# wasiahmad/context_attentive_ir

Measured on AMD Instinct MI355X. Metric: ranked (query,doc) pairs/sec, higher is better.
Workload: dtype f32; 1 GPU; cars, batch=16 sessions x session_len 7 x 10 candidates, q_len=4, doc_len=64, emb_dim=300, vocab=100000, f32, full-length Zipf ids; macro_batch=8, lanes=4, batches_in_flight=32, hipgraph=True, parallelism=single GPU, world_size=1

## Files before the change

### context_attentive_ir_amd/csrc/cars_attn.hip

```cpp
#include <algorithm>
#include <mutex>
#include <type_traits>
#include "common.hpp"

namespace nir {

typedef _Float16 f16x8 __attribute__((ext_vector_type(8)));
typedef __fp16 fp16x2_t __attribute__((ext_vector_type(2)));
typedef float f32x4 __attribute__((ext_vector_type(4)));

constexpr int AP_D = 256;
constexpr int AP_ROWS = 64, AP_RT = 4, AP_CT = 4, AP_S = AP_D / 32;
constexpr int AP_KG = AP_ROWS * 8 + 32;
constexpr int AP_PLANE_HALVES = 2 * AP_S * 4 * AP_KG;
constexpr int AP_RED_FLOATS = 4 * 16 * AP_D;
constexpr size_t AP_LDS = (size_t)(AP_PLANE_HALVES * 2 > AP_RED_FLOATS * 4 ? AP_PLANE_HALVES * 2 : AP_RED_FLOATS * 4) + (4 * 64 + 64) * 4;

#define AP_MMA(ACC, A, W) asm volatile("v_mfma_f32_16x16x32_f16 %0, %1, %2, %0" : "+a"(ACC) : "v"(A), "v"(W))
#define AP_MMA_DRAIN() asm volatile("s_nop 15\n\ts_nop 15" ::: "memory")

__device__ __forceinline__ void ap_mma_n(int n, f32x4 (&acc)[AP_CT][AP_RT], f32x4 (&acx)[AP_CT][AP_RT], const f16x8 (&af)[AP_RT][2],
                                         const f16x8 (&w)[AP_CT][2]) {
    const int j = n / (3 * AP_RT), ph = (n / AP_RT) % 3, i = n % AP_RT;
    if (ph == 0) AP_MMA(acx[j][i], af[i][1], w[j][0]);
// ... 8 lines not shown
    if (T >= 16) v = fmaxf(v, dpp_mov<0x140>(v));
    if (T >= 32) v = fmaxf(v, __shfl_xor(v, 16));
    if (T >= 64) v = fmaxf(v, __shfl_xor(v, 32));
    return v;
}
__device__ __forceinline__ float ap_group_sum(float v, int T) {
    v += dpp_mov<0xB1>(v);
    v += dpp_mov<0x4E>(v);
    if (T >= 8) v += dpp_mov<0x141>(v);
    if (T >= 16) v += dpp_mov<0x140>(v);
    if (T >= 32) v += __shfl_xor(v, 16);
    if (T >= 64) v += __shfl_xor(v, 32);
    return v;
}

struct AttnPoolArgs {
    const float* h;
    const _Float16* wf;
    const float *b0, *w3, *b3;
    const int64_t* lens;
    float* pooled;
    int64_t M;
    int T, logT;
    int io_prio;
};

__global__ __launch_bounds__(256, 1) void attn_pool_fused_kernel(AttnPoolArgs p) {
    extern __shared__ __attribute__((aligned(16))) unsigned short asm_[];
    unsigned short* Pp = asm_;
    float* rowpart = reinterpret_cast<float*>(asm_ + (AP_LDS - (4 * 64 + 64) * 4) / 2);
    float* prob = rowpart + 4 * 64;
    constexpr int KG = AP_KG;
    const int tid = threadIdx.x, lane = tid & 63, wave = tid >> 6;
    const int g = lane >> 4, c16 = lane & 15;
    const int T = p.T;
    const int64_t row0 = (int64_t)blockIdx.x * AP_ROWS, nrows = p.M * T;

    const _Float16* wp = p.wf + ((int64_t)(AP_CT * wave) * 2 * 64 + lane) * 8;
    constexpr int WSTEP = 16 * 2 * 64 * 8;
    f16x8 w[AP_CT][2], wb[AP_CT][2], afa[AP_RT][2], afb[AP_RT][2];
    {
        float4 hv[16];
#pragma unroll
        for (int j = 0; j < 16; ++j) {
            int64_t r = row0 + wave + 4 * j;
            r = r < nrows ? r : nrows - 1;
            hv[j] = *reinterpret_cast<const float4*>(p.h + r * AP_D + 4 * lane);
// ... 125 lines not shown
            a.x = fmaf(pr, hv[j].x, a.x); a.y = fmaf(pr, hv[j].y, a.y); a.z = fmaf(pr, hv[j].z, a.z); a.w = fmaf(pr, hv[j].w, a.w);
            if (((j + 1) & (per - 1)) == 0) {
                red[(wave * RS + (j >> (p.logT - 2))) * 64 + lane] = a;
                a = make_float4(0.f, 0.f, 0.f, 0.f);
            }
        }
        __syncthreads();
        for (int idx = tid; idx < RS * 64; idx += 256) {
            const int q = idx >> 6, c = idx & 63;
            const int64_t seq = (row0 >> p.logT) + q;
            if (seq < p.M) {
                const float4 a0 = red[(0 * RS + q) * 64 + c], a1 = red[(1 * RS + q) * 64 + c], a2 = red[(2 * RS + q) * 64 + c],
                             a3 = red[(3 * RS + q) * 64 + c];
                float4 o;
                o.x = (a0.x + a1.x) + (a2.x + a3.x); o.y = (a0.y + a1.y) + (a2.y + a3.y);
                o.z = (a0.z + a1.z) + (a2.z + a3.z); o.w = (a0.w + a1.w) + (a2.w + a3.w);
                *reinterpret_cast<float4*>(p.pooled + seq * AP_D + 4 * c) = o;
            }
        }
    }
}

#ifdef AP_TIMING
__device__ long long ap_dbg[16];
#define AP_T(I) if (blockIdx.x == 7 && lane == 0 && it == 5) ap_dbg[I] = __builtin_readcyclecounter();
#else
#define AP_T(I)
#endif
constexpr int AP2_KG = AP_ROWS * 8;
constexpr int AP2_PLANE_HALVES = 2 * AP_S * 4 * AP2_KG;
constexpr size_t AP2_LDS = (size_t)2 * AP2_PLANE_HALVES * 2 + (2 * 4 * 64 + 4 * 64 + 2 * AP_D) * 4;

template <bool ONE, bool ROW1>
__device__ __forceinline__ void ap2_mma_n(int n, f32x4 (&acc)[AP_CT][AP_RT], f32x4 (&acx)[AP_CT][AP_RT], const f16x8 (&af)[AP_RT][2],
                                          const f16x8 (&w)[AP_CT][2]) {
    const int i = n / (3 * AP_CT), ph = (n / AP_CT) % 3, j = n % AP_CT;
    if (ph == 2) AP_MMA(acc[j][i], af[i][0], w[j][0]);
    else if (ONE) return;
    else if (ph == 0) { if (!ROW1) AP_MMA(acx[j][i], af[i][1], w[j][0]); }
    else AP_MMA(acx[j][i], af[i][0], w[j][1]);
}

#ifndef AP_FMAMIX
#define AP_FMAMIX 1
#endif
__device__ __forceinline__ void ap_fma_mix(float4& a, const uint2 u, const float s) {
    asm volatile("v_fma_mix_f32 %0, %1, %2, %0 op_sel:[0,0,0] op_sel_hi:[1,0,0]" : "+v"(a.x) : "v"(u.x), "v"(s));
    asm volatile("v_fma_mix_f32 %0, %1, %2, %0 op_sel:[1,0,0] op_sel_hi:[1,0,0]" : "+v"(a.y) : "v"(u.x), "v"(s));
    asm volatile("v_fma_mix_f32 %0, %1, %2, %0 op_sel:[0,0,0] op_sel_hi:[1,0,0]" : "+v"(a.z) : "v"(u.y), "v"(s));
    asm volatile("v_fma_mix_f32 %0, %1, %2, %0 op_sel:[1,0,0] op_sel_hi:[1,0,0]" : "+v"(a.w) : "v"(u.y), "v"(s));
}

template <bool ONE, int IN>
__global__ __launch_bounds__(512, 1) void attn_pool_pipe_kernel(AttnPoolArgs p, int64_t ntiles) {
    constexpr bool IN16 = IN == 1;
    constexpr bool ROW1 = ONE || IN16;
    extern __shared__ __attribute__((aligned(16))) unsigned short asm2_[];
    constexpr int KG = AP2_KG, PH = AP2_PLANE_HALVES;
    float* rowpart = reinterpret_cast<float*>(asm2_ + 2 * PH);
    float* probw = rowpart + 2 * 4 * 64;
    float* bw = probw + 4 * 64;
    const int tid = threadIdx.x, lane = tid & 63, wave = tid >> 6, w4 = wave & 3;
    if (tid < AP_D) bw[tid] = p.b0[tid] * 2.8853900817779268f;
    else bw[tid] = p.w3[tid - AP_D];
    __syncthreads();
    const bool mma_role = wave < 4;
    const int g = lane >> 4, c16 = lane & 15;
    const int T = p.T;
    const int64_t nrows = p.M * T;
    const int64_t G = gridDim.x;
    const int64_t nk = (ntiles - blockIdx.x + G - 1) / G;

    if (mma_role) {
        __builtin_amdgcn_s_setprio(3);
        const _Float16* wbase = p.wf + (int64_t)(AP_CT * __builtin_amdgcn_readfirstlane(w4)) * 2 * 64 * 8;
        uint32_t wlane = (uint32_t)lane * 16u;
        auto ldw = [&](int off_halves) {
            return *reinterpret_cast<const f16x8*>(reinterpret_cast<const char*>(wbase + off_halves) + (uint64_t)wlane);
        };
        constexpr int WSTEP = 16 * 2 * 64 * 8;
        const int foff_e = g * KG + (c16 ^ (2 * (g >> 1))) * 8, foff_o = g * KG + (c16 ^ (4 + 2 * (g >> 1))) * 8;
        f16x8 wa[AP_CT][2], wb[AP_CT][2], af[AP_RT][2];
        f32x4 acc[AP_CT][AP_RT], acx[AP_CT][AP_RT];
#pragma unroll
        for (int j = 0; j < AP_CT; ++j) {
            wa[j][0] = ldw((j * 2) * 512);
            wa[j][1] = ONE ? wa[j][0] : ldw((j * 2 + 1) * 512);
        }
        for (int64_t it = 0; it < nk + 2; ++it) {
            if (w4 == 0) { AP_T(0) }
            if (it >= 1 && it <= nk) {
                const unsigned short* Pp = asm2_ + ((it - 1) & 1) * PH;
                float* rp = rowpart + ((it - 1) & 1) * 4 * 64;
#pragma unroll
                for (int j = 0; j < AP_CT; ++j)
#pragma unroll
                    for (int i = 0; i < AP_RT; ++i) {
                        acc[j][i] = f32x4{0.f, 0.f, 0.f, 0.f};
                        acx[j][i] = f32x4{0.f, 0.f, 0.f, 0.f};
                    }
#pragma unroll
                for (int i = 0; i < AP_RT - 1; ++i) {
                    af[i][0] = *reinterpret_cast<const f16x8*>(Pp + foff_e + i * 128);
                    af[i][1] = *reinterpret_cast<const f16x8*>(Pp + AP_S * 4 * KG + foff_e + i * 128);
                }
#define AP2_STEP(S, WC, WN, LAST, ODD)                                                    \
                {                                                                         \
                    const int sn_ = ((S) + 1) & (AP_S - 1);                               \
                    asm volatile("" : "+v"(wlane));                                       \
                    const unsigned short* pc_ = Pp + (S) * 4 * KG + ((ODD) ? foff_o : foff_e);  \
                    const unsigned short* pn_ = Pp + sn_ * 4 * KG + ((ODD) ? foff_e : foff_o);  \
                    _Pragma("clang loop unroll(full)") for (int n_ = 0; n_ < 3 * AP_RT * AP_CT; ++n_) { \
                        ap2_mma_n<ONE, ROW1>(n_, acc, acx, af, WC);                             \
                        if (n_ % 6 == 2 && n_ / 6 < 2 * AP_CT && !(ONE && ((n_ / 6) & 1))) {  \
                            asm volatile("" ::"v"(WN[(n_ / 6) >> 1][(n_ / 6) & 1]));      \
                            WN[(n_ / 6) >> 1][(n_ / 6) & 1] = ldw(sn_ * WSTEP + (n_ / 6) * 512);  \
                        }                                                                 \
                        if (n_ == 7 || n_ == 8) {                                         \
                            asm volatile("" ::"v"(af[3][n_ - 7]));                        \
                            af[3][n_ - 7] = *reinterpret_cast<const f16x8*>(pc_ + (n_ - 7) * AP_S * 4 * KG + 3 * 128); \
                        }                                                                 \
                        if (!(LAST) && n_ >= 19 && (n_ - 19) % 12 < 2 && (n_ - 19) / 12 < AP_RT - 1) { \
                            asm volatile("" ::"v"(af[(n_ - 19) / 12][(n_ - 19) % 12]));   \
                            af[(n_ - 19) / 12][(n_ - 19) % 12] =                          \
                                *reinterpret_cast<const f16x8*>(pn_ + ((n_ - 19) % 12) * AP_S * 4 * KG + ((n_ - 19) / 12) * 128); \
                        }                                                                 \
                        __builtin_amdgcn_sched_barrier(0);                                \
                    }                                                                     \
                    _Pragma("unroll") for (int j_ = 0; j_ < AP_CT; ++j_) asm volatile("" ::"v"(WC[j_][0]), "v"(WC[j_][1])); \
                    _Pragma("unroll") for (int i_ = 0; i_ < AP_RT; ++i_) asm volatile("" ::"v"(af[i_][0]), "v"(af[i_][1])); \
                }
#pragma unroll 1
                for (int s = 0; s < AP_S - 2; s += 2) {
                    AP2_STEP(s, wa, wb, 0, 0)
                    AP2_STEP(s + 1, wb, wa, 0, 1)
                }
                AP2_STEP(AP_S - 2, wa, wb, 0, 0)
                AP2_STEP(AP_S - 1, wb, wa, 1, 1)
                if (w4 == 0) { AP_T(1) }
                AP_MMA_DRAIN();
                {
                    constexpr float C2 = 2.8853900817779268f;
                    float rs[AP_RT][4], bzv[AP_CT], w3v[AP_CT];
#pragma unroll
                    for (int j = 0; j < AP_CT; ++j) {
                        const int col = 64 * w4 + 16 * j + c16;
                        bzv[j] = bw[col];
                        w3v[j] = bw[AP_D + col];
                    }
                    const float r0 = -0.5f * ((w3v[0] + w3v[1]) + (w3v[2] + w3v[3]));
#pragma unroll
                    for (int i = 0; i < AP_RT; ++i)
#pragma unroll
                        for (int r = 0; r < 4; ++r) rs[i][r] = r0;
#pragma unroll
                    for (int j = 0; j < AP_CT; ++j) {
#pragma unroll
                        for (int i = 0; i < AP_RT; ++i)
#pragma unroll
                            for (int r = 0; r < 4; ++r) {
                                const float z = fmaf(fmaf(acx[j][i][r], 1.0f / 2048.0f, acc[j][i][r]), C2, bzv[j]);
                                rs[i][r] = fmaf(w3v[j], __builtin_amdgcn_rcpf(1.0f + __builtin_amdgcn_exp2f(z)), rs[i][r]);
                            }
                    }
#pragma unroll
                    for (int i = 0; i < AP_RT; ++i)
#pragma unroll
                        for (int r = 0; r < 4; ++r) {
                            float v = rs[i][r];
                            v += dpp_mov<0xB1>(v);
                            v += dpp_mov<0x4E>(v);
                            v += dpp_mov<0x141>(v);
                            v += dpp_mov<0x140>(v);
                            if (c16 == 0) rp[w4 * 64 + 16 * i + 4 * g + r] = -2.0f * v;
                        }
                }
            }
            if (w4 == 0) { AP_T(2) }
            __syncthreads();
            if (w4 == 0) { AP_T(3) }
        }
    } else {
        if (p.io_prio) __builtin_amdgcn_s_setprio(2);
        float* pw = probw + w4 * 64;
        const int sub = lane >> 4, per = T / 4;
        const int col = 64 * w4 + 4 * c16;
        const int poff = ((col >> 5) * 4 + ((col >> 3) & 3)) * KG + (col & 7);
        const int xq = c16 >> 3, sx = sub ^ (2 * ((c16 >> 2) & 1));
        const int roff_e = (4 * xq + sx) * 8, roff_o = (4 * (1 ^ xq) + sx) * 8;
        float4 ld[IN16 ? 1 : 16];
        uint2 ld16[IN16 ? 16 : 1];
        const float b3v = p.b3[0];
        int len_ld = T, len_1 = T, len_2 = T;
        auto load_rows = [&](int64_t k) {
            const int64_t row0 = (blockIdx.x + k * G) * AP_ROWS;
            {
                const int64_t seq = (row0 + lane) >> p.logT;
                len_ld = T;
                if (p.lens) len_ld = (int)p.lens[seq < p.M ? seq : p.M - 1];
            }
#pragma unroll
            for (int q = 0; q < 16; ++q) {
                int64_t r = row0 + 4 * q + sub;
                r = r < nrows ? r : nrows - 1;
                if (IN16) ld16[q] = *reinterpret_cast<const uint2*>(reinterpret_cast<const _Float16*>(p.h) + r * AP_D + col);
                else ld[q] = *reinterpret_cast<const float4*>(p.h + r * AP_D + col);
            }
        };
        if (nk > 0) load_rows(0);
        for (int64_t it = 0; it < nk + 2; ++it) {
            unsigned short* Pb = asm2_ + (it & 1) * PH + poff;
            unsigned short* Pbe = Pb + roff_e;
            unsigned short* Pbo = Pb + roff_o;
            if (w4 == 0) { AP_T(4) }
            if (it >= 2) {
                const int64_t rowS = (blockIdx.x + (it - 2) * G) * AP_ROWS;
                const float* rp = rowpart + (it & 1) * 4 * 64;
                {
                    const int64_t r = rowS + lane;
                    const int64_t seq = r >> p.logT;
                    const int t = (int)(r - seq * T);
                    int len = len_2;
                    len = len < 0 ? 0 : (len > T ? T : len);
                    const bool ok = seq < p.M && t < len;
                    const float lg = (rp[lane] + rp[64 + lane]) + (rp[128 + lane] + rp[192 + lane]) + b3v;
                    const float mx = ap_group_max(ok ? lg : -INFINITY, T);
                    const float e = ok ? __expf(lg - mx) : 0.f;
                    const float den = ap_group_sum(e, T);
                    pw[lane] = e / den;
                    asm volatile("s_waitcnt lgkmcnt(0)" ::: "memory");
                }
                if (w4 == 0) { AP_T(8) }
                float4 a = make_float4(0.f, 0.f, 0.f, 0.f);
#pragma unroll
                for (int hb = 0; hb < 2; ++hb) {
                    uint2 u1[8], u2[ROW1 ? 1 : 8];
                    float prr[8];
#pragma unroll
                    for (int q8 = 0; q8 < 8; ++q8) {
                        const int row = 4 * (8 * hb + q8) + sub;
                        const unsigned short* src = ((q8 & 1) ? Pbo : Pbe) + ((8 * hb + q8) >> 1) * 64;
                        u1[q8] = *reinterpret_cast<const uint2*>(src);
                        if (!ROW1) u2[q8] = *reinterpret_cast<const uint2*>(src + AP_S * 4 * KG);
                        prr[q8] = pw[row];
                    }
#pragma unroll
                    for (int q8 = 0; q8 < 8; ++q8) {
                        const int q = 8 * hb + q8;
                        const fp16x2_t a01 = __builtin_bit_cast(fp16x2_t, u1[q8].x), a23 = __builtin_bit_cast(fp16x2_t, u1[q8].y);
                        const float pr = prr[q8];
#if AP_FMAMIX
                        (void)a01; (void)a23;
                        ap_fma_mix(a, u1[q8], pr);
                        if (!ROW1) ap_fma_mix(a, u2[q8], pr * (1.0f / 2048.0f));
#else
                        if (ROW1) {
                            a.x = fmaf(pr, (float)a01[0], a.x);
                            a.y = fmaf(pr, (float)a01[1], a.y);
                            a.z = fmaf(pr, (float)a23[0], a.z);
                            a.w = fmaf(pr, (float)a23[1], a.w);
                        } else {
                            const fp16x2_t b01 = __builtin_bit_cast(fp16x2_t, u2[q8].x), b23 = __builtin_bit_cast(fp16x2_t, u2[q8].y);
                            a.x = fmaf(pr, fmaf((float)b01[0], 1.0f / 2048.0f, (float)a01[0]), a.x);
                            a.y = fmaf(pr, fmaf((float)b01[1], 1.0f / 2048.0f, (float)a01[1]), a.y);
                            a.z = fmaf(pr, fmaf((float)b23[0], 1.0f / 2048.0f, (float)a23[0]), a.z);
                            a.w = fmaf(pr, fmaf((float)b23[1], 1.0f / 2048.0f, (float)a23[1]), a.w);
                        }
#endif
                        if (((q + 1) & (per - 1)) == 0) {
                            a.x += __shfl_xor(a.x, 16); a.y += __shfl_xor(a.y, 16); a.z += __shfl_xor(a.z, 16); a.w += __shfl_xor(a.w, 16);
                            a.x += __shfl_xor(a.x, 32); a.y += __shfl_xor(a.y, 32); a.z += __shfl_xor(a.z, 32); a.w += __shfl_xor(a.w, 32);
                            const int64_t seq = (rowS >> p.logT) + (q >> (p.logT - 2));
                            if (sub == 0 && seq < p.M) *reinterpret_cast<float4*>(p.pooled + seq * AP_D + col) = a;
                            a = make_float4(0.f, 0.f, 0.f, 0.f);
                        }
                    }
                }
            }
            if (w4 == 0) { AP_T(5) }
            if (it < nk) {
#pragma unroll
                for (int q = 0; q < 16; ++q) {
                    unsigned short* d = ((q & 1) ? Pbo : Pbe) + (q >> 1) * 64;
                    if (IN16) {
                        *reinterpret_cast<uint2*>(d) = ld16[q];
                        continue;
                    }
                    const float4 v = ld[q];
                    if (IN == 2) {
                        *reinterpret_cast<uint2*>(d) = make_uint2(__float_as_uint(v.x), __float_as_uint(v.y));
                        *reinterpret_cast<uint2*>(d + AP_S * 4 * KG) = make_uint2(__float_as_uint(v.z), __float_as_uint(v.w));
                        continue;
                    }
                    const fp16x2_t a01 = __builtin_amdgcn_cvt_pkrtz(v.x, v.y), a23 = __builtin_amdgcn_cvt_pkrtz(v.z, v.w);
                    *reinterpret_cast<uint2*>(d) = make_uint2(__builtin_bit_cast(unsigned, a01), __builtin_bit_cast(unsigned, a23));
                    if (!ONE) {
                        const fp16x2_t b01 = __builtin_amdgcn_cvt_pkrtz((v.x - (float)a01[0]) * 2048.0f, (v.y - (float)a01[1]) * 2048.0f);
                        const fp16x2_t b23 = __builtin_amdgcn_cvt_pkrtz((v.z - (float)a23[0]) * 2048.0f, (v.w - (float)a23[1]) * 2048.0f);
                        *reinterpret_cast<uint2*>(d + AP_S * 4 * KG) = make_uint2(__builtin_bit_cast(unsigned, b01), __builtin_bit_cast(unsigned, b23));
                    }
                }
                if (w4 == 0) { AP_T(6) }
                len_2 = len_1;
                len_1 = len_ld;
                if (it + 1 < nk) load_rows(it + 1);
            } else {
                len_2 = len_1;
            }
            if (w4 == 0) { AP_T(7) }
            __syncthreads();
        }
    }
}

#ifdef AP_TIMING
}
extern "C" int nir_debug_attn_timing(long long* out16) { return (int)hipMemcpyFromSymbol(out16, HIP_SYMBOL(nir::ap_dbg), sizeof(long long) * 16); }
namespace nir {
#endif

bool attn_pool_fused_usable(int D, int T) { return D == AP_D && (T == 4 || T == 8 || T == 16 || T == 32 || T == 64); }

static int ap_cu_count() {
    static const int ncu = [] {
        int dev = 0;
        hipDeviceProp_t prop;
        return (hipGetDevice(&dev) == hipSuccess && hipGetDeviceProperties(&prop, dev) == hipSuccess && prop.multiProcessorCount > 0)
                   ? prop.multiProcessorCount : 256;
    }();
    return ncu;
}
bool attn_pool_pipe_selected(int64_t M, int T) {
    const int64_t tiles = (M * T + AP_ROWS - 1) / AP_ROWS;
    const int pipe = tun(g_tun.attn_unfused_pipe);
    return (tiles >= 2 * (int64_t)ap_cu_count() && pipe == 0) || pipe == 2;
}

int launch_attn_pool_fused(const float* h, const void* wfrag, const float* b0, const float* w3, const float* b3, const int64_t* lens, int64_t M,
                           int T, float* pooled, int one_term, hipStream_t st, int in_f16) {
    NIR_REQUIRE(h && wfrag && b0 && w3 && b3 && pooled && attn_pool_fused_usable(AP_D, T), "attn_pool_fused: bad args (T=%d)", T);
    if (M == 0) return 0;
    AttnPoolArgs a;
    a.h = h; a.wf = (const _Float16*)wfrag; a.b0 = b0; a.w3 = w3; a.b3 = b3; a.lens = lens; a.pooled = pooled; a.M = M; a.T = T; a.logT = __builtin_ctz((unsigned)T);
    a.io_prio = tun(g_tun.attn_io_prio);
    static std::once_flag once;
    std::call_once(once, [] { (void)hipFuncSetAttribute((const void*)attn_pool_fused_kernel, hipFuncAttributeMaxDynamicSharedMemorySize, (int)AP_LDS); });
    const int64_t tiles = (M * T + AP_ROWS - 1) / AP_ROWS;
    const bool pipe_sel = attn_pool_pipe_selected(M, T);
    const char* pname = !pipe_sel ? "attn_pool_fused_kernel" : in_f16 == 1 ? "attn_pool_pipe_kernel<true,1>" : in_f16 == 3 ? "attn_pool_pipe_kernel<false,1>" :
                        in_f16 == 2 ? "attn_pool_pipe_kernel<false,2>" :
                        one_term ? "attn_pool_pipe_kernel<true,0>" : "attn_pool_pipe_kernel<false,0>";
    ProfScope ps(prof_shape_name(pname, M * T, AP_D, AP_D), st);
    static std::once_flag once2;
    std::call_once(once2, [] {
        (void)hipFuncSetAttribute((const void*)attn_pool_pipe_kernel<false, 0>, hipFuncAttributeMaxDynamicSharedMemorySize, (int)AP2_LDS);
        (void)hipFuncSetAttribute((const void*)attn_pool_pipe_kernel<false, 2>, hipFuncAttributeMaxDynamicSharedMemorySize, (int)AP2_LDS);
        (void)hipFuncSetAttribute((const void*)attn_pool_pipe_kernel<true, 0>, hipFuncAttributeMaxDynamicSharedMemorySize, (int)AP2_LDS);
        (void)hipFuncSetAttribute((const void*)attn_pool_pipe_kernel<true, 1>, hipFuncAttributeMaxDynamicSharedMemorySize, (int)AP2_LDS);
        (void)hipFuncSetAttribute((const void*)attn_pool_pipe_kernel<false, 1>, hipFuncAttributeMaxDynamicSharedMemorySize, (int)AP2_LDS);
    });
    const int ncu = ap_cu_count();
    if (pipe_sel) {
        const dim3 grid((unsigned)std::min<int64_t>(tiles, ncu));
        NIR_REQUIRE(in_f16 != 2 || !one_term, "attn_pool_fused: term-pair rows come from the fp32-accurate encoder (two terms)");
        if (in_f16 == 1) hipLaunchKernelGGL((attn_pool_pipe_kernel<true, 1>), grid, dim3(512), AP2_LDS, st, a, tiles);
        else if (in_f16 == 3) hipLaunchKernelGGL((attn_pool_pipe_kernel<false, 1>), grid, dim3(512), AP2_LDS, st, a, tiles);
        else if (in_f16 == 2) hipLaunchKernelGGL((attn_pool_pipe_kernel<false, 2>), grid, dim3(512), AP2_LDS, st, a, tiles);
// ... 12 lines not shown
```

### context_attentive_ir_amd/csrc/common.hpp

```cpp
#pragma once
#include <hip/hip_runtime.h>
#include <stdint.h>
#include <stdio.h>
#include <stdarg.h>
#include <atomic>
#include "../../include/neuroir_hip.h"

namespace nir {

void set_error(const char* fmt, ...);

#define NIR_REQUIRE(cond, ...)                 \
    do {                                       \
        if (!(cond)) {                         \
            nir::set_error(__VA_ARGS__);       \
            return NIR_ERR_BAD_ARG;            \
        }                                      \
    } while (0)

#define NIR_CHECK_LAUNCH(name)                                                      \
    do {                                                                            \
        hipError_t e__ = hipGetLastError();                                         \
        if (e__ != hipSuccess) {                                                    \
            nir::set_error("%s: launch failed: %s", name, hipGetErrorString(e__)); \
// ... 10 lines not shown
struct ProfScope {
    void* rec;
    hipStream_t st;
    ProfScope(const char* name, hipStream_t stream);
    ~ProfScope();
};

const char* prof_shape_name(const char* base, long long M, long long N, long long K);

struct ForkJoin {
    hipStream_t main, side;
    hipEvent_t ev_fork, ev_join;
    bool ok, open;
    explicit ForkJoin(hipStream_t main_stream);
    ~ForkJoin() { if (open) join(); }
    void fork();
    void join();
};

extern unsigned long long* g_debug_buf;
int batches_in_flight(hipStream_t st);

struct Tunables {
    std::atomic<int> no_fork, lstm_mfma16, lstm_s, debug, exact_f32, duet_unfused, attn_unfused, attn_unfused_pipe, duet_rows64, attn_fp32_rows, attn_io_prio, cl_poll_limit;
};
extern Tunables g_tun;
inline int tun(const std::atomic<int>& a) { return a.load(std::memory_order_relaxed); }

constexpr int WAVE = 64;

template <int CTRL>
__device__ __forceinline__ float dpp_mov(float v) {
    return __builtin_bit_cast(float, __builtin_amdgcn_update_dpp(0, __builtin_bit_cast(int, v), CTRL, 0xF, 0xF, true));
}
__device__ __forceinline__ float readlane_f(float v, int lane) {
    return __builtin_bit_cast(float, __builtin_amdgcn_readlane(__builtin_bit_cast(int, v), lane));
}
__device__ __forceinline__ float wave_sum(float v) {
    v += dpp_mov<0xB1>(v);
    v += dpp_mov<0x4E>(v);
    v += dpp_mov<0x141>(v);
    v += dpp_mov<0x140>(v);
    return (readlane_f(v, 0) + readlane_f(v, 16)) + (readlane_f(v, 32) + readlane_f(v, 48));
}
__device__ __forceinline__ float wave_max(float v) {
    v = fmaxf(v, dpp_mov<0xB1>(v));
    v = fmaxf(v, dpp_mov<0x4E>(v));
// ... 94 lines not shown
```

### context_attentive_ir_amd/csrc/core.hip

```cpp
#include "common.hpp"
#include <string.h>
#include <stdlib.h>
#include <atomic>
#include <map>
#include <mutex>
#include <string>
#include <vector>

namespace nir {
static thread_local char g_err[512] = "";
void set_error(const char* fmt, ...) {
    va_list ap;
    va_start(ap, fmt);
    vsnprintf(g_err, sizeof(g_err), fmt, ap);
    va_end(ap);
}
}

namespace nir {
struct ProfRec { const char* name; hipEvent_t a, b; };
static std::mutex g_prof_mu;
static std::vector<ProfRec*> g_prof;
static std::atomic<int> g_prof_on{0};

// ... 113 lines not shown
static int env_flag(const char* name) { return getenv(name) ? 1 : 0; }
Tunables g_tun{{env_flag("NIR_NO_FORK")}, {env_int("NIR_LSTM_MFMA16", -1)}, {env_int("NIR_LSTM_S", 0)}, {env_flag("NIR_DEBUG")},
               {env_flag("NIR_EXACT_F32")}};
}
extern "C" int nir_set_stream_batches_in_flight(nir_stream_t stream, int n) {
    std::lock_guard<std::mutex> lk(nir::g_bif_mu);
    if (n < 1) nir::g_bif_map.erase((hipStream_t)stream);
    else nir::g_bif_map[(hipStream_t)stream] = n;
    nir::g_bif_streams.store((int)nir::g_bif_map.size());
    return 0;
}
static const bool g_tunables_mutable = getenv("NIR_DEBUG_TUNABLES") != nullptr;
extern "C" int nir_debug_set_tunable(const char* name, int value) {
    using namespace nir;
    if (!name) return NIR_ERR_BAD_ARG;
    if (!g_tunables_mutable) {
        set_error("nir_debug_set_tunable('%s'): the switches are frozen at load time; set NIR_DEBUG_TUNABLES=1 before loading the library (debug / test processes only)", name);
        return NIR_ERR_BAD_ARG;
    }
    struct { const char* n; std::atomic<int>* a; } tab[] = {
        {"no_fork", &g_tun.no_fork}, {"lstm_mfma16", &g_tun.lstm_mfma16}, {"lstm_s", &g_tun.lstm_s}, {"debug", &g_tun.debug},
        {"exact_f32", &g_tun.exact_f32}, {"duet_unfused", &g_tun.duet_unfused}, {"attn_unfused", &g_tun.attn_unfused},
        {"attn_unfused_pipe", &g_tun.attn_unfused_pipe}, {"duet_rows64", &g_tun.duet_rows64}, {"attn_fp32_rows", &g_tun.attn_fp32_rows},
        {"attn_io_prio", &g_tun.attn_io_prio}, {"cl_poll_limit", &g_tun.cl_poll_limit}};
    for (auto& t : tab)
        if (!strcmp(t.n, name)) { t.a->store(value); return 0; }
    set_error("nir_debug_set_tunable: unknown tunable '%s'", name);
    return NIR_ERR_BAD_ARG;
}
extern "C" int nir_debug_set_buffer(void* dev_u64) { nir::g_debug_buf = (unsigned long long*)dev_u64; return 0; }

__global__ void clock_probe_kernel(unsigned long long* out, int iters, float* sink) {
    extern __shared__ float probe_lds[];
    unsigned long long c0 = clock64(), w0 = wall_clock64();
    if (iters < 0) probe_lds[threadIdx.x] = 1.f;
    float a = threadIdx.x * 1e-9f, b = 1.000001f;
    for (int i = 0; i < iters; ++i) a = fmaf(a, b, 1e-7f);
    unsigned long long c1 = clock64(), w1 = wall_clock64();
    if (a == 123.456f) sink[0] = a;
    if (blockIdx.x == 0 && threadIdx.x == 0) { out[0] = c1 - c0; out[1] = w1 - w0; }
    if (threadIdx.x == 0 && blockIdx.x < 2048) {
        out[2 + 3 * blockIdx.x] = w0;
        out[3 + 3 * blockIdx.x] = w1;
        out[4 + 3 * blockIdx.x] = __builtin_amdgcn_s_getreg(63492);
    }
}
extern "C" int nir_debug_clock_probe(void* out, int iters, int blocks, void* sink, nir_stream_t stream) {
// ... 198 lines not shown
```

Before: 8.325 million pairs/s.

## Restructure attention-pool pipe kernel into two symmetric ping-pong wave groups

The pipelined attention-pool kernel previously split waves into dedicated MFMA waves and I/O/softmax waves. Now two groups of four waves each own one LDS plane and alternate tiles. Each group runs MFMA, scoring, softmax, pooling and staging of its next tile, with an LDS atomic counter for intra-group sync and shared barriers between groups. The goal is to overlap one group's MFMA phase with the other's memory and epilogue work without a fixed role imbalance. The cost is more complex synchronisation and a higher register load per wave. The unused io_prio tunable is also removed.

```diff
diff --git a/context_attentive_ir_amd/csrc/cars_attn.hip b/context_attentive_ir_amd/csrc/cars_attn.hip
--- a/context_attentive_ir_amd/csrc/cars_attn.hip
+++ b/context_attentive_ir_amd/csrc/cars_attn.hip
@@ -54,7 +54,6 @@
     float* pooled;
     int64_t M;
     int T, logT;
-    int io_prio;
 };
 
 __global__ __launch_bounds__(256, 1) void attn_pool_fused_kernel(AttnPoolArgs p) {
@@ -226,14 +225,16 @@
 }
 
 #ifdef AP_TIMING
-__device__ long long ap_dbg[16];
-#define AP_T(I) if (blockIdx.x == 7 && lane == 0 && it == 5) ap_dbg[I] = __builtin_readcyclecounter();
+__device__ long long ap_dbg[32];
+#define AP_T(I) if (blockIdx.x == 7 && lane == 0 && w4 == 0 && (it >> 1) == 3) ap_dbg[grp * 16 + (I)] = __builtin_readcyclecounter();
+#define AP_TM(I) if (blockIdx.x == 7 && lane == 0 && w4 == 0 && (it >> 1) == 2) ap_dbg[grp * 16 + (I)] = __builtin_readcyclecounter();
 #else
 #define AP_T(I)
+#define AP_TM(I)
 #endif
 constexpr int AP2_KG = AP_ROWS * 8;
 constexpr int AP2_PLANE_HALVES = 2 * AP_S * 4 * AP2_KG;
-constexpr size_t AP2_LDS = (size_t)2 * AP2_PLANE_HALVES * 2 + (2 * 4 * 64 + 4 * 64 + 2 * AP_D) * 4;
+constexpr size_t AP2_LDS = (size_t)2 * AP2_PLANE_HALVES * 2 + (2 * 4 * 64 + 8 * 64 + 2 * AP_D + 4) * 4;
 
 template <bool ONE, bool ROW1>
 __device__ __forceinline__ void ap2_mma_n(int n, f32x4 (&acc)[AP_CT][AP_RT], f32x4 (&acx)[AP_CT][AP_RT], const f16x8 (&af)[AP_RT][2],
@@ -245,6 +246,9 @@
     else AP_MMA(acx[j][i], af[i][0], w[j][1]);
 }
 
+#ifndef AP_WSUM_ROWS
+#define AP_WSUM_ROWS 4
+#endif
 #ifndef AP_FMAMIX
 #define AP_FMAMIX 1
 #endif
@@ -255,6 +259,17 @@
     asm volatile("v_fma_mix_f32 %0, %1, %2, %0 op_sel:[1,0,0] op_sel_hi:[1,0,0]" : "+v"(a.w) : "v"(u.y), "v"(s));
 }
 
+#ifdef AP_ACC_ASM
+#define AP_ACC(A, R) ap_acc(A, R)
+#else
+#define AP_ACC(A, R) (A)[R]
+#endif
+__device__ __forceinline__ float ap_acc(const f32x4& a, int r) {
+    float x;
+    asm volatile("v_accvgpr_read_b32 %0, %1" : "=v"(x) : "a"(a[r]));
+    return x;
+}
+
 template <bool ONE, int IN>
 __global__ __launch_bounds__(512, 1) void attn_pool_pipe_kernel(AttnPoolArgs p, int64_t ntiles) {
     constexpr bool IN16 = IN == 1;
@@ -263,263 +278,291 @@
     constexpr int KG = AP2_KG, PH = AP2_PLANE_HALVES;
     float* rowpart = reinterpret_cast<float*>(asm2_ + 2 * PH);
     float* probw = rowpart + 2 * 4 * 64;
-    float* bw = probw + 4 * 64;
-    const int tid = threadIdx.x, lane = tid & 63, wave = tid >> 6, w4 = wave & 3;
+    float* bw = probw + 8 * 64;
+    unsigned* arrived = reinterpret_cast<unsigned*>(bw + 2 * AP_D);
+    const int tid = threadIdx.x, lane = tid & 63, wave = tid >> 6, w4 = wave & 3, grp = wave >> 2;
     if (tid < AP_D) bw[tid] = p.b0[tid] * 2.8853900817779268f;
     else bw[tid] = p.w3[tid - AP_D];
+    if (tid < 2) arrived[tid] = 0u;
     __syncthreads();
-    const bool mma_role = wave < 4;
     const int g = lane >> 4, c16 = lane & 15;
     const int T = p.T;
     const int64_t nrows = p.M * T;
     const int64_t G = gridDim.x;
     const int64_t nk = (ntiles - blockIdx.x + G - 1) / G;
-
-    if (mma_role) {
-        __builtin_amdgcn_s_setprio(3);
-        const _Float16* wbase = p.wf + (int64_t)(AP_CT * __builtin_amdgcn_readfirstlane(w4)) * 2 * 64 * 8;
-        uint32_t wlane = (uint32_t)lane * 16u;
-        auto ldw = [&](int off_halves) {
-            return *reinterpret_cast<const f16x8*>(reinterpret_cast<const char*>(wbase + off_halves) + (uint64_t)wlane);
-        };
-        constexpr int WSTEP = 16 * 2 * 64 * 8;
-        const int foff_e = g * KG + (c16 ^ (2 * (g >> 1))) * 8, foff_o = g * KG + (c16 ^ (4 + 2 * (g >> 1))) * 8;
-        f16x8 wa[AP_CT][2], wb[AP_CT][2], af[AP_RT][2];
-        f32x4 acc[AP_CT][AP_RT], acx[AP_CT][AP_RT];
+    unsigned short* const Pp = asm2_ + grp * PH;
+    float* const rp = rowpart + grp * 4 * 64;
+
+    const _Float16* wbase = p.wf + (int64_t)(AP_CT * __builtin_amdgcn_readfirstlane(w4)) * 2 * 64 * 8;
+    uint32_t wlane = (uint32_t)lane * 16u;
+    auto ldw = [&](int off_halves) {
+        return *reinterpret_cast<const f16x8*>(reinterpret_cast<const char*>(wbase + off_halves) + (uint64_t)wlane);
+    };
+    constexpr int WSTEP = 16 * 2 * 64 * 8;
+    const int foff_e = g * KG + (c16 ^ (2 * (g >> 1))) * 8, foff_o = g * KG + (c16 ^ (4 + 2 * (g >> 1))) * 8;
+    f16x8 wa[AP_CT][2], wb[AP_CT][2], af[AP_RT][2];
+    f32x4 acc[AP_CT][AP_RT], acx[AP_CT][AP_RT];
+
+    float* pw = probw + wave * 64;
+    const int sub = g, per = T / 4;
+    const int col = 64 * w4 + 4 * c16;
+    const int poff = ((col >> 5) * 4 + ((col >> 3) & 3)) * KG + (col & 7);
+    const int xq = c16 >> 3, sx = sub ^ (2 * ((c16 >> 2) & 1));
+    unsigned short* const Pbe = Pp + poff + (4 * xq + sx) * 8;
+    unsigned short* const Pbo = Pp + poff + (4 * (1 ^ xq) + sx) * 8;
+    float4 ld[IN16 ? 1 : 16];
+    uint2 ld16[IN16 ? 16 : 1];
+    const float b3v = p.b3[0];
+    int len_ld = T, len_fin = T;
+    auto load_rows = [&](int64_t k) {
+        const int64_t row0 = (blockIdx.x + k * G) * AP_ROWS;
+        {
+            const int64_t seq = (row0 + lane) >> p.logT;
+            len_ld = T;
+            if (p.lens) len_ld = (int)p.lens[seq < p.M ? seq : p.M - 1];
+        }
+#pragma unroll
+        for (int q = 0; q < 16; ++q) {
+            int64_t r = row0 + 4 * q + sub;
+            r = r < nrows ? r : nrows - 1;
+            if (IN16) ld16[q] = *reinterpret_cast<const uint2*>(reinterpret_cast<const _Float16*>(p.h) + r * AP_D + col);
+            else ld[q] = *reinterpret_cast<const float4*>(p.h + r * AP_D + col);
+        }
+    };
+
+    auto stage_tile = [&]() {
+        asm volatile("" ::: "memory");
+        __builtin_amdgcn_sched_barrier(0);
+#pragma unroll
+        for (int q = 0; q < 16; ++q) {
+            unsigned short* d = ((q & 1) ? Pbo : Pbe) + (q >> 1) * 64;
+            if (IN16) {
+                *reinterpret_cast<uint2*>(d) = ld16[q];
+                continue;
+            }
+            const float4 v = ld[q];
+            if (IN == 2) {
+                *reinterpret_cast<uint2*>(d) = make_uint2(__float_as_uint(v.x), __float_as_uint(v.y));
+                *reinterpret_cast<uint2*>(d + AP_S * 4 * KG) = make_uint2(__float_as_uint(v.z), __float_as_uint(v.w));
+                continue;
+            }
+            const fp16x2_t a01 = __builtin_amdgcn_cvt_pkrtz(v.x, v.y), a23 = __builtin_amdgcn_cvt_pkrtz(v.z, v.w);
+            *reinterpret_cast<uint2*>(d) = make_uint2(__builtin_bit_cast(unsigned, a01), __builtin_bit_cast(unsigned, a23));
+            if (!ONE) {
+                const fp16x2_t b01 = __builtin_amdgcn_cvt_pkrtz((v.x - (float)a01[0]) * 2048.0f, (v.y - (float)a01[1]) * 2048.0f);
+                const fp16x2_t b23 = __builtin_amdgcn_cvt_pkrtz((v.z - (float)a23[0]) * 2048.0f, (v.w - (float)a23[1]) * 2048.0f);
+                *reinterpret_cast<uint2*>(d + AP_S * 4 * KG) = make_uint2(__builtin_bit_cast(unsigned, b01), __builtin_bit_cast(unsigned, b23));
+            }
+        }
+        len_fin = len_ld;
+        asm volatile("" ::: "memory");
+        __builtin_amdgcn_sched_barrier(0);
 #pragma unroll
         for (int j = 0; j < AP_CT; ++j) {
             wa[j][0] = ldw((j * 2) * 512);
             wa[j][1] = ONE ? wa[j][0] : ldw((j * 2 + 1) * 512);
         }
-        for (int64_t it = 0; it < nk + 2; ++it) {
-            if (w4 == 0) { AP_T(0) }
-            if (it >= 1 && it <= nk) {
-                const unsigned short* Pp = asm2_ + ((it - 1) & 1) * PH;
-                float* rp = rowpart + ((it - 1) & 1) * 4 * 64;
-#pragma unroll
-                for (int j = 0; j < AP_CT; ++j)
-#pragma unroll
-                    for (int i = 0; i < AP_RT; ++i) {
-                        acc[j][i] = f32x4{0.f, 0.f, 0.f, 0.f};
-                        acx[j][i] = f32x4{0.f, 0.f, 0.f, 0.f};
+    };
+    int64_t it = grp;
+    if (grp) __syncthreads();
+    if (it < nk) {
+        load_rows(it);
+        stage_tile();
+    }
+    __syncthreads();
+    for (;;) {
+        if (it >= nk) {
+            if (it == nk) __syncthreads();
+            break;
+        }
+        __builtin_amdgcn_s_setprio(3);
+#pragma unroll
+        for (int j = 0; j < AP_CT; ++j)
+#pragma unroll
+            for (int i = 0; i < AP_RT; ++i) {
+                acc[j][i] = f32x4{0.f, 0.f, 0.f, 0.f};
+                acx[j][i] = f32x4{0.f, 0.f, 0.f, 0.f};
+            }
+#pragma unroll
+        for (int j = 0; j < AP_CT; ++j) asm volatile("" : "=v"(wb[j][0]), "=v"(wb[j][1]));
+        asm volatile("" : "=v"(af[AP_RT - 1][0]), "=v"(af[AP_RT - 1][1]));
+#pragma unroll
+        for (int i = 0; i < AP_RT - 1; ++i) {
+            af[i][0] = *reinterpret_cast<const f16x8*>(Pp + foff_e + i * 128);
+            af[i][1] = *reinterpret_cast<const f16x8*>(Pp + AP_S * 4 * KG + foff_e + i * 128);
+        }
+#define AP2_STEP(S, WC, WN, LAST, ODD)                                                    \
+        {                                                                             \
+            const int sn_ = ((S) + 1) & (AP_S - 1);                                   \
+            asm volatile("" : "+v"(wlane));                                           \
+            const unsigned short* pc_ = Pp + (S) * 4 * KG + ((ODD) ? foff_o : foff_e);  \
+            const unsigned short* pn_ = Pp + sn_ * 4 * KG + ((ODD) ? foff_e : foff_o);  \
+            _Pragma("clang loop unroll(full)") for (int n_ = 0; n_ < 3 * AP_RT * AP_CT; ++n_) { \
+                ap2_mma_n<ONE, ROW1>(n_, acc, acx, af, WC);                           \
+                if (!(LAST) && n_ % 6 == 2 && n_ / 6 < 2 * AP_CT && !(ONE && ((n_ / 6) & 1))) {  \
+                    asm volatile("" ::"v"(WN[(n_ / 6) >> 1][(n_ / 6) & 1]));          \
+                    WN[(n_ / 6) >> 1][(n_ / 6) & 1] = ldw(sn_ * WSTEP + (n_ / 6) * 512);  \
+                }                                                                     \
+                if (n_ == 7 || n_ == 8) {                                             \
+                    asm volatile("" ::"v"(af[3][n_ - 7]));                            \
+                    af[3][n_ - 7] = *reinterpret_cast<const f16x8*>(pc_ + (n_ - 7) * AP_S * 4 * KG + 3 * 128); \
+                }                                                                     \
+                if (!(LAST) && n_ >= 19 && (n_ - 19) % 12 < 2 && (n_ - 19) / 12 < AP_RT - 1) { \
+                    asm volatile("" ::"v"(af[(n_ - 19) / 12][(n_ - 19) % 12]));       \
+                    af[(n_ - 19) / 12][(n_ - 19) % 12] =                              \
+                        *reinterpret_cast<const f16x8*>(pn_ + ((n_ - 19) % 12) * AP_S * 4 * KG + ((n_ - 19) / 12) * 128); \
+                }                                                                     \
+                __builtin_amdgcn_sched_barrier(0);                                    \
+            }                                                                         \
+            _Pragma("unroll") for (int j_ = 0; j_ < AP_CT; ++j_) asm volatile("" ::"v"(WC[j_][0]), "v"(WC[j_][1])); \
+            _Pragma("unroll") for (int i_ = 0; i_ < AP_RT; ++i_) asm volatile("" ::"v"(af[i_][0]), "v"(af[i_][1])); \
+        }
+#pragma unroll 1
+        for (int s = 0; s < AP_S - 2; s += 2) {
+            AP2_STEP(s, wa, wb, 0, 0)
+            AP2_STEP(s + 1, wb, wa, 0, 1)
+        }
+        AP2_STEP(AP_S - 2, wa, wb, 0, 0)
+        AP2_STEP(AP_S - 1, wb, wa, 1, 1)
+        AP_TM(1)
+        AP_MMA_DRAIN();
+        __syncthreads();
+        it += 2;
+        __builtin_amdgcn_s_setprio(0);
+        const bool stage = it < nk;
+        const int len_use = len_fin;
+        AP_T(2)
+#pragma unroll
+        for (int q = 0; q < (IN16 ? 1 : 16); ++q) asm volatile("" : "=v"(ld[q]));
+#pragma unroll
+        for (int q = 0; q < (IN16 ? 16 : 1); ++q) asm volatile("" : "=v"(ld16[q]));
+        if (stage) load_rows(it);
+        asm volatile("" ::: "memory");
+        __builtin_amdgcn_sched_barrier(0);
+        AP_T(3)
+        const int64_t rowS = (blockIdx.x + (it - 2) * G) * AP_ROWS;
+        {
+            constexpr float C2 = 2.8853900817779268f;
+            float rs[AP_RT][4], bzv[AP_CT], w3v[AP_CT];
+#pragma unroll
+            for (int j = 0; j < AP_CT; ++j) {
+                const int cc = 64 * w4 + 16 * j + c16;
+                bzv[j] = bw[cc];
+                w3v[j] = bw[AP_D + cc];
+            }
+            const float r0 = -0.5f * ((w3v[0] + w3v[1]) + (w3v[2] + w3v[3]));
+#pragma unroll
+            for (int i = 0; i < AP_RT; ++i)
+#pragma unroll
+                for (int r = 0; r < 4; ++r) rs[i][r] = r0;
+#pragma unroll
+            for (int j = 0; j < AP_CT; ++j) {
+#pragma unroll
+                for (int i = 0; i < AP_RT; ++i) {
+#pragma unroll
+                    for (int r = 0; r < 4; ++r) {
+                        const float z = fmaf(fmaf(AP_ACC(acx[j][i], r), 1.0f / 2048.0f, AP_ACC(acc[j][i], r)), C2, bzv[j]);
+                        rs[i][r] = fmaf(w3v[j], __builtin_amdgcn_rcpf(1.0f + __builtin_amdgcn_exp2f(z)), rs[i][r]);
                     }
-#pragma unroll
-                for (int i = 0; i < AP_RT - 1; ++i) {
-                    af[i][0] = *reinterpret_cast<const f16x8*>(Pp + foff_e + i * 128);
-                    af[i][1] = *reinterpret_cast<const f16x8*>(Pp + AP_S * 4 * KG + foff_e + i * 128);
+                    __builtin_amdgcn_sched_barrier(0);
                 }
-#define AP2_STEP(S, WC, WN, LAST, ODD)                                                    \
-                {                                                                         \
-                    const int sn_ = ((S) + 1) & (AP_S - 1);                               \
-                    asm volatile("" : "+v"(wlane));                                       \
-                    const unsigned short* pc_ = Pp + (S) * 4 * KG + ((ODD) ? foff_o : foff_e);  \
-                    const unsigned short* pn_ = Pp + sn_ * 4 * KG + ((ODD) ? foff_e : foff_o);  \
-                    _Pragma("clang loop unroll(full)") for (int n_ = 0; n_ < 3 * AP_RT * AP_CT; ++n_) { \
-                        ap2_mma_n<ONE, ROW1>(n_, acc, acx, af, WC);                             \
-                        if (n_ % 6 == 2 && n_ / 6 < 2 * AP_CT && !(ONE && ((n_ / 6) & 1))) {  \
-                            asm volatile("" ::"v"(WN[(n_ / 6) >> 1][(n_ / 6) & 1]));      \
-                            WN[(n_ / 6) >> 1][(n_ / 6) & 1] = ldw(sn_ * WSTEP + (n_ / 6) * 512);  \
-                        }                                                                 \
-                        if (n_ == 7 || n_ == 8) {                                         \
-                            asm volatile("" ::"v"(af[3][n_ - 7]));                        \
-                            af[3][n_ - 7] = *reinterpret_cast<const f16x8*>(pc_ + (n_ - 7) * AP_S * 4 * KG + 3 * 128); \
-                        }                                                                 \
-                        if (!(LAST) && n_ >= 19 && (n_ - 19) % 12 < 2 && (n_ - 19) / 12 < AP_RT - 1) { \
-                            asm volatile("" ::"v"(af[(n_ - 19) / 12][(n_ - 19) % 12]));   \
-                            af[(n_ - 19) / 12][(n_ - 19) % 12] =                          \
-                                *reinterpret_cast<const f16x8*>(pn_ + ((n_ - 19) % 12) * AP_S * 4 * KG + ((n_ - 19) / 12) * 128); \
-                        }                                                                 \
-                        __builtin_amdgcn_sched_barrier(0);                                \
-                    }                                                                     \
-                    _Pragma("unroll") for (int j_ = 0; j_ < AP_CT; ++j_) asm volatile("" ::"v"(WC[j_][0]), "v"(WC[j_][1])); \
-                    _Pragma("unroll") for (int i_ = 0; i_ < AP_RT; ++i_) asm volatile("" ::"v"(af[i_][0]), "v"(af[i_][1])); \
+            }
+#pragma unroll
+            for (int i = 0; i < AP_RT; ++i)
+#pragma unroll
+                for (int r = 0; r < 4; ++r) {
+                    float v = rs[i][r];
+                    v += dpp_mov<0xB1>(v);
+                    v += dpp_mov<0x4E>(v);
+                    v += dpp_mov<0x141>(v);
+                    v += dpp_mov<0x140>(v);
+                    if (c16 == 0) rp[w4 * 64 + 16 * i + 4 * g + r] = -2.0f * v;
                 }
-#pragma unroll 1
-                for (int s = 0; s < AP_S - 2; s += 2) {
-                    AP2_STEP(s, wa, wb, 0, 0)
-                    AP2_STEP(s + 1, wb, wa, 0, 1)
+        }
+        asm volatile("s_waitcnt lgkmcnt(0)" ::: "memory");
+        if (lane == 0) __hip_atomic_fetch_add(arrived + grp, 1u, __ATOMIC_RELAXED, __HIP_MEMORY_SCOPE_WORKGROUP);
+        AP_T(4)
+        {
+            const unsigned want = 4u * (unsigned)(((it - 2) >> 1) + 1);
+            while (__builtin_amdgcn_readfirstlane(__hip_atomic_load(arrived + grp, __ATOMIC_RELAXED, __HIP_MEMORY_SCOPE_WORKGROUP)) < want)
+                __builtin_amdgcn_s_sleep(1);
+            asm volatile("" ::: "memory");
+        }
+        AP_T(5)
+        {
+            const int64_t r = rowS + lane;
+            const int64_t seq = r >> p.logT;
+            const int t = (int)(r - seq * T);
+            int len = len_use;
+            len = len < 0 ? 0 : (len > T ? T : len);
+            const bool ok = seq < p.M && t < len;
+            const float lg = (rp[lane] + rp[64 + lane]) + (rp[128 + lane] + rp[192 + lane]) + b3v;
+            const float mx = ap_group_max(ok ? lg : -INFINITY, T);
+            const float e = ok ? __expf(lg - mx) : 0.f;
+            const float den = ap_group_sum(e, T);
+            pw[lane] = e / den;
+            asm volatile("s_waitcnt lgkmcnt(0)" ::: "memory");
+        }
+        AP_T(6)
+        constexpr int WB = AP_WSUM_ROWS;
+        float4 a = make_float4(0.f, 0.f, 0.f, 0.f);
+#pragma unroll
+        for (int hb = 0; hb < 16 / WB; ++hb) {
+            uint2 u1[WB], u2[ROW1 ? 1 : WB];
+            float prr[WB];
+#pragma unroll
+            for (int q8 = 0; q8 < WB; ++q8) {
+                const int row = 4 * (WB * hb + q8) + sub;
+                const unsigned short* src = ((q8 & 1) ? Pbo : Pbe) + ((WB * hb + q8) >> 1) * 64;
+                u1[q8] = *reinterpret_cast<const uint2*>(src);
+                if (!ROW1) u2[q8] = *reinterpret_cast<const uint2*>(src + AP_S * 4 * KG);
+                prr[q8] = pw[row];
+            }
+#pragma unroll
+            for (int q8 = 0; q8 < WB; ++q8) {
+                const int q = WB * hb + q8;
+                const fp16x2_t a01 = __builtin_bit_cast(fp16x2_t, u1[q8].x), a23 = __builtin_bit_cast(fp16x2_t, u1[q8].y);
+                const float pr = prr[q8];
+#if AP_FMAMIX
+                (void)a01; (void)a23;
+                ap_fma_mix(a, u1[q8], pr);
+                if (!ROW1) ap_fma_mix(a, u2[q8], pr * (1.0f / 2048.0f));
+#else
+                if (ROW1) {
+                    a.x = fmaf(pr, (float)a01[0], a.x);
+                    a.y = fmaf(pr, (float)a01[1], a.y);
+                    a.z = fmaf(pr, (float)a23[0], a.z);
+                    a.w = fmaf(pr, (float)a23[1], a.w);
+                } else {
+                    const fp16x2_t b01 = __builtin_bit_cast(fp16x2_t, u2[q8].x), b23 = __builtin_bit_cast(fp16x2_t, u2[q8].y);
+                    a.x = fmaf(pr, fmaf((float)b01[0], 1.0f / 2048.0f, (float)a01[0]), a.x);
+                    a.y = fmaf(pr, fmaf((float)b01[1], 1.0f / 2048.0f, (float)a01[1]), a.y);
+                    a.z = fmaf(pr, fmaf((float)b23[0], 1.0f / 2048.0f, (float)a23[0]), a.z);
+                    a.w = fmaf(pr, fmaf((float)b23[1], 1.0f / 2048.0f, (float)a23[1]), a.w);
                 }
-                AP2_STEP(AP_S - 2, wa, wb, 0, 0)
-                AP2_STEP(AP_S - 1, wb, wa, 1, 1)
-                if (w4 == 0) { AP_T(1) }
-                AP_MMA_DRAIN();
-                {
-                    constexpr float C2 = 2.8853900817779268f;
-                    float rs[AP_RT][4], bzv[AP_CT], w3v[AP_CT];
-#pragma unroll
-                    for (int j = 0; j < AP_CT; ++j) {
-                        const int col = 64 * w4 + 16 * j + c16;
-                        bzv[j] = bw[col];
-                        w3v[j] = bw[AP_D + col];
-                    }
-                    const float r0 = -0.5f * ((w3v[0] + w3v[1]) + (w3v[2] + w3v[3]));
-#pragma unroll
-                    for (int i = 0; i < AP_RT; ++i)
-#pragma unroll
-                        for (int r = 0; r < 4; ++r) rs[i][r] = r0;
-#pragma unroll
-                    for (int j = 0; j < AP_CT; ++j) {
-#pragma unroll
-                        for (int i = 0; i < AP_RT; ++i)
-#pragma unroll
-                            for (int r = 0; r < 4; ++r) {
-                                const float z = fmaf(fmaf(acx[j][i][r], 1.0f / 2048.0f, acc[j][i][r]), C2, bzv[j]);
-                                rs[i][r] = fmaf(w3v[j], __builtin_amdgcn_rcpf(1.0f + __builtin_amdgcn_exp2f(z)), rs[i][r]);
-                            }
-                    }
-#pragma unroll
-                    for (int i = 0; i < AP_RT; ++i)
-#pragma unroll
-                        for (int r = 0; r < 4; ++r) {
-                            float v = rs[i][r];
-                            v += dpp_mov<0xB1>(v);
-                            v += dpp_mov<0x4E>(v);
-                            v += dpp_mov<0x141>(v);
-                            v += dpp_mov<0x140>(v);
-                            if (c16 == 0) rp[w4 * 64 + 16 * i + 4 * g + r] = -2.0f * v;
-                        }
+#endif
+                if (((q + 1) & (per - 1)) == 0) {
+                    a.x += __shfl_xor(a.x, 16); a.y += __shfl_xor(a.y, 16); a.z += __shfl_xor(a.z, 16); a.w += __shfl_xor(a.w, 16);
+                    a.x += __shfl_xor(a.x, 32); a.y += __shfl_xor(a.y, 32); a.z += __shfl_xor(a.z, 32); a.w += __shfl_xor(a.w, 32);
+                    const int64_t seq = (rowS >> p.logT) + (q >> (p.logT - 2));
+                    if (sub == 0 && seq < p.M) *reinterpret_cast<float4*>(p.pooled + seq * AP_D + col) = a;
+                    a = make_float4(0.f, 0.f, 0.f, 0.f);
                 }
             }
-            if (w4 == 0) { AP_T(2) }
-            __syncthreads();
-            if (w4 == 0) { AP_T(3) }
-        }
-    } else {
-        if (p.io_prio) __builtin_amdgcn_s_setprio(2);
-        float* pw = probw + w4 * 64;
-        const int sub = lane >> 4, per = T / 4;
-        const int col = 64 * w4 + 4 * c16;
-        const int poff = ((col >> 5) * 4 + ((col >> 3) & 3)) * KG + (col & 7);
-        const int xq = c16 >> 3, sx = sub ^ (2 * ((c16 >> 2) & 1));
-        const int roff_e = (4 * xq + sx) * 8, roff_o = (4 * (1 ^ xq) + sx) * 8;
-        float4 ld[IN16 ? 1 : 16];
-        uint2 ld16[IN16 ? 16 : 1];
-        const float b3v = p.b3[0];
-        int len_ld = T, len_1 = T, len_2 = T;
-        auto load_rows = [&](int64_t k) {
-            const int64_t row0 = (blockIdx.x + k * G) * AP_ROWS;
-            {
-                const int64_t seq = (row0 + lane) >> p.logT;
-                len_ld = T;
-                if (p.lens) len_ld = (int)p.lens[seq < p.M ? seq : p.M - 1];
-            }
-#pragma unroll
-            for (int q = 0; q < 16; ++q) {
-                int64_t r = row0 + 4 * q + sub;
-                r = r < nrows ? r : nrows - 1;
-                if (IN16) ld16[q] = *reinterpret_cast<const uint2*>(reinterpret_cast<const _Float16*>(p.h) + r * AP_D + col);
-                else ld[q] = *reinterpret_cast<const float4*>(p.h + r * AP_D + col);
-            }
-        };
-        if (nk > 0) load_rows(0);
-        for (int64_t it = 0; it < nk + 2; ++it) {
-            unsigned short* Pb = asm2_ + (it & 1) * PH + poff;
-            unsigned short* Pbe = Pb + roff_e;
-            unsigned short* Pbo = Pb + roff_o;
-            if (w4 == 0) { AP_T(4) }
-            if (it >= 2) {
-                const int64_t rowS = (blockIdx.x + (it - 2) * G) * AP_ROWS;
-                const float* rp = rowpart + (it & 1) * 4 * 64;
-                {
-                    const int64_t r = rowS + lane;
-                    const int64_t seq = r >> p.logT;
-                    const int t = (int)(r - seq * T);
-                    int len = len_2;
-                    len = len < 0 ? 0 : (len > T ? T : len);
-                    const bool ok = seq < p.M && t < len;
-                    const float lg = (rp[lane] + rp[64 + lane]) + (rp[128 + lane] + rp[192 + lane]) + b3v;
-                    const float mx = ap_group_max(ok ? lg : -INFINITY, T);
-                    const float e = ok ? __expf(lg - mx) : 0.f;
-                    const float den = ap_group_sum(e, T);
-                    pw[lane] = e / den;
-                    asm volatile("s_waitcnt lgkmcnt(0)" ::: "memory");
-                }
-                if (w4 == 0) { AP_T(8) }
-                float4 a = make_float4(0.f, 0.f, 0.f, 0.f);
-#pragma unroll
-                for (int hb = 0; hb < 2; ++hb) {
-                    uint2 u1[8], u2[ROW1 ? 1 : 8];
-                    float prr[8];
-#pragma unroll
-                    for (int q8 = 0; q8 < 8; ++q8) {
-                        const int row = 4 * (8 * hb + q8) + sub;
-                        const unsigned short* src = ((q8 & 1) ? Pbo : Pbe) + ((8 * hb + q8) >> 1) * 64;
-                        u1[q8] = *reinterpret_cast<const uint2*>(src);
-                        if (!ROW1) u2[q8] = *reinterpret_cast<const uint2*>(src + AP_S * 4 * KG);
-                        prr[q8] = pw[row];
-                    }
-#pragma unroll
-                    for (int q8 = 0; q8 < 8; ++q8) {
-                        const int q = 8 * hb + q8;
-                        const fp16x2_t a01 = __builtin_bit_cast(fp16x2_t, u1[q8].x), a23 = __builtin_bit_cast(fp16x2_t, u1[q8].y);
-                        const float pr = prr[q8];
-#if AP_FMAMIX
-                        (void)a01; (void)a23;
-                        ap_fma_mix(a, u1[q8], pr);
-                        if (!ROW1) ap_fma_mix(a, u2[q8], pr * (1.0f / 2048.0f));
-#else
-                        if (ROW1) {
-                            a.x = fmaf(pr, (float)a01[0], a.x);
-                            a.y = fmaf(pr, (float)a01[1], a.y);
-                            a.z = fmaf(pr, (float)a23[0], a.z);
-                            a.w = fmaf(pr, (float)a23[1], a.w);
-                        } else {
-                            const fp16x2_t b01 = __builtin_bit_cast(fp16x2_t, u2[q8].x), b23 = __builtin_bit_cast(fp16x2_t, u2[q8].y);
-                            a.x = fmaf(pr, fmaf((float)b01[0], 1.0f / 2048.0f, (float)a01[0]), a.x);
-                            a.y = fmaf(pr, fmaf((float)b01[1], 1.0f / 2048.0f, (float)a01[1]), a.y);
-                            a.z = fmaf(pr, fmaf((float)b23[0], 1.0f / 2048.0f, (float)a23[0]), a.z);
-                            a.w = fmaf(pr, fmaf((float)b23[1], 1.0f / 2048.0f, (float)a23[1]), a.w);
-                        }
-#endif
-                        if (((q + 1) & (per - 1)) == 0) {
-                            a.x += __shfl_xor(a.x, 16); a.y += __shfl_xor(a.y, 16); a.z += __shfl_xor(a.z, 16); a.w += __shfl_xor(a.w, 16);
-                            a.x += __shfl_xor(a.x, 32); a.y += __shfl_xor(a.y, 32); a.z += __shfl_xor(a.z, 32); a.w += __shfl_xor(a.w, 32);
-                            const int64_t seq = (rowS >> p.logT) + (q >> (p.logT - 2));
-                            if (sub == 0 && seq < p.M) *reinterpret_cast<float4*>(p.pooled + seq * AP_D + col) = a;
-                            a = make_float4(0.f, 0.f, 0.f, 0.f);
-                        }
-                    }
-                }
-            }
-            if (w4 == 0) { AP_T(5) }
-            if (it < nk) {
-#pragma unroll
-                for (int q = 0; q < 16; ++q) {
-                    unsigned short* d = ((q & 1) ? Pbo : Pbe) + (q >> 1) * 64;
-                    if (IN16) {
-                        *reinterpret_cast<uint2*>(d) = ld16[q];
-                        continue;
-                    }
-                    const float4 v = ld[q];
-                    if (IN == 2) {
-                        *reinterpret_cast<uint2*>(d) = make_uint2(__float_as_uint(v.x), __float_as_uint(v.y));
-                        *reinterpret_cast<uint2*>(d + AP_S * 4 * KG) = make_uint2(__float_as_uint(v.z), __float_as_uint(v.w));
-                        continue;
-                    }
-                    const fp16x2_t a01 = __builtin_amdgcn_cvt_pkrtz(v.x, v.y), a23 = __builtin_amdgcn_cvt_pkrtz(v.z, v.w);
-                    *reinterpret_cast<uint2*>(d) = make_uint2(__builtin_bit_cast(unsigned, a01), __builtin_bit_cast(unsigned, a23));
-                    if (!ONE) {
-                        const fp16x2_t b01 = __builtin_amdgcn_cvt_pkrtz((v.x - (float)a01[0]) * 2048.0f, (v.y - (float)a01[1]) * 2048.0f);
-                        const fp16x2_t b23 = __builtin_amdgcn_cvt_pkrtz((v.z - (float)a23[0]) * 2048.0f, (v.w - (float)a23[1]) * 2048.0f);
-                        *reinterpret_cast<uint2*>(d + AP_S * 4 * KG) = make_uint2(__builtin_bit_cast(unsigned, b01), __builtin_bit_cast(unsigned, b23));
-                    }
-                }
-                if (w4 == 0) { AP_T(6) }
-                len_2 = len_1;
-                len_1 = len_ld;
-                if (it + 1 < nk) load_rows(it + 1);
-            } else {
-                len_2 = len_1;
-            }
-            if (w4 == 0) { AP_T(7) }
-            __syncthreads();
-        }
+        }
+        AP_T(7)
+#pragma unroll
+        for (int j = 0; j < AP_CT; ++j) asm volatile("" : "=v"(wa[j][0]), "=v"(wa[j][1]));
+        if (stage) stage_tile();
+        AP_T(8)
+        __syncthreads();
+        AP_T(9)
     }
 }
 
 #ifdef AP_TIMING
 }
-extern "C" int nir_debug_attn_timing(long long* out16) { return (int)hipMemcpyFromSymbol(out16, HIP_SYMBOL(nir::ap_dbg), sizeof(long long) * 16); }
+extern "C" int nir_debug_attn_timing(long long* out32) { return (int)hipMemcpyFromSymbol(out32, HIP_SYMBOL(nir::ap_dbg), sizeof(long long) * 32); }
 namespace nir {
 #endif
 
@@ -546,7 +589,6 @@
     if (M == 0) return 0;
     AttnPoolArgs a;
     a.h = h; a.wf = (const _Float16*)wfrag; a.b0 = b0; a.w3 = w3; a.b3 = b3; a.lens = lens; a.pooled = pooled; a.M = M; a.T = T; a.logT = __builtin_ctz((unsigned)T);
-    a.io_prio = tun(g_tun.attn_io_prio);
     static std::once_flag once;
     std::call_once(once, [] { (void)hipFuncSetAttribute((const void*)attn_pool_fused_kernel, hipFuncAttributeMaxDynamicSharedMemorySize, (int)AP_LDS); });
     const int64_t tiles = (M * T + AP_ROWS - 1) / AP_ROWS;
diff --git a/context_attentive_ir_amd/csrc/common.hpp b/context_attentive_ir_amd/csrc/common.hpp
--- a/context_attentive_ir_amd/csrc/common.hpp
+++ b/context_attentive_ir_amd/csrc/common.hpp
@@ -56,7 +56,7 @@
 int batches_in_flight(hipStream_t st);
 
 struct Tunables {
-    std::atomic<int> no_fork, lstm_mfma16, lstm_s, debug, exact_f32, duet_unfused, attn_unfused, attn_unfused_pipe, duet_rows64, attn_fp32_rows, attn_io_prio, cl_poll_limit;
+    std::atomic<int> no_fork, lstm_mfma16, lstm_s, debug, exact_f32, duet_unfused, attn_unfused, attn_unfused_pipe, duet_rows64, attn_fp32_rows, cl_poll_limit;
 };
 extern Tunables g_tun;
 inline int tun(const std::atomic<int>& a) { return a.load(std::memory_order_relaxed); }
diff --git a/context_attentive_ir_amd/csrc/core.hip b/context_attentive_ir_amd/csrc/core.hip
--- a/context_attentive_ir_amd/csrc/core.hip
+++ b/context_attentive_ir_amd/csrc/core.hip
@@ -159,7 +159,7 @@
         {"no_fork", &g_tun.no_fork}, {"lstm_mfma16", &g_tun.lstm_mfma16}, {"lstm_s", &g_tun.lstm_s}, {"debug", &g_tun.debug},
         {"exact_f32", &g_tun.exact_f32}, {"duet_unfused", &g_tun.duet_unfused}, {"attn_unfused", &g_tun.attn_unfused},
         {"attn_unfused_pipe", &g_tun.attn_unfused_pipe}, {"duet_rows64", &g_tun.duet_rows64}, {"attn_fp32_rows", &g_tun.attn_fp32_rows},
-        {"attn_io_prio", &g_tun.attn_io_prio}, {"cl_poll_limit", &g_tun.cl_poll_limit}};
+        {"cl_poll_limit", &g_tun.cl_poll_limit}};
     for (auto& t : tab)
         if (!strcmp(t.n, name)) { t.a->store(value); return 0; }
     set_error("nir_debug_set_tunable: unknown tunable '%s'", name);
```

New measurement: 6.566 million pairs/s, median of 2. 0.789x the previous value.
